# davide-coccomini/MINTIME-Multi-Identity-size-iNvariant-TIMEsformer-for-Video-Deepfake-Detection

Measured on AMD Instinct MI355X. Metric: clips/sec (8-frame, 2-identity, 224^2 crops) fwd+bwd, higher is better.
Workload: dtype f32; 1 GPU; config 3: EfficientNet-B0 + SizeInvariantTimeSformer(dim 512, depth 9, heads 8), B=32/GPU, 8 frames, 2 identities (identity-masked), 224x224 crops, random-init seeded weights (restored before every step), train-mode BN + drop-connect 0.2, step = fwd + BCE loss + bwd + SGD(lr .01, wd 1e-4); global_batch=32, frames=8, parallelism=dp1

## Files before the change

### include/mintime_hip.h

```cpp
#ifndef MINTIME_HIP_H
#define MINTIME_HIP_H
#include <stdint.h>
#ifdef __cplusplus
extern "C" {
#endif

#define MT_VERSION 122

int mt_version(void);
const char* mt_last_error(void);

int mt_set_deterministic(int on);
int mt_get_deterministic(void);
int mt_det_release(void* stream);
int mt_det_bn_sums(const float* x, const float* z, const float* mean_invstd, int64_t rows, int C, int mode, double* stats, void* stream);

typedef struct { int gin, gout, off; } mt_rowmap;

enum { MT_OP_NT = 0,
       MT_OP_NN = 1,
       MT_OP_TN = 2 };

enum { MT_PRO_NONE = 0, MT_PRO_BN_SWISH_GATE = 1, MT_PRO_BN_SWISH = 2, MT_PRO_AFFINE = 3,
       MT_PRO_BN_BWD = 4,
// ... 38 lines not shown
int mt_gemm_set_precision(int level);
int mt_gemm_get_precision(void);

int mt_split_planes(const float* src, void* planes, int64_t n, void* stream);

int64_t mt_planes_elems(int rows, int cols);

int mt_split_planes_blk(const float* src, int64_t ld, int rows, int cols, void* planes, void* stream);

int mt_split_planes_blk_multi(const void* items, int count, int64_t total_blocks, void* stream);

int mt_bn_bwd_apply_planes(const float* du, const float* z, const float* kabc, void* planes, int rows, int C, void* stream);

typedef struct {
  int op;
  int epilogue;
  int M, N, K;
  const void* a_planes;
  const void* b_planes;
  float* C; int64_t ldc;
  const float* bias;
  const float* R; int64_t ldr;
  float* C2; int64_t ldc2;
  int n_half;
  float* col_sum;
  void* c_planes;
  int split_k;
  void* sk_workspace;
  int64_t sk_workspace_bytes;
  double* stats; int stats_slots;
} mt_gemm_planes_desc;

int mt_gemm_planes(const mt_gemm_planes_desc* d, void* stream);

int mt_mul_planes(const float* x, const float* m, void* planes, float* out, int rows, int cols, void* stream);
int mt_mul_add(const float* y, const float* m, const float* r, float* out, int64_t n, void* stream);
int mt_geglu_bwd(const float* dh, const float* m, const float* u, void* du_planes, float* du, int rows, int n_half, void* stream);
int64_t mt_gemm_planes_workspace_bytes(void);
int mt_gemm_planes_set_persist(int blocks_per_cu);


int mt_layernorm_fwd(const float* x, const float* gamma, const float* beta, float* y, float* stats,
                     int rows, int dim, float eps, void* y_planes, void* stream);

int mt_embed_fwd(float* x, const float* cls, const float* pos_emb, const float* size_emb,
                 const int64_t* positions, const int32_t* sizes, int B, int F, int n, int dim, int pos_rows, int size_rows,
                 int* err_flag, void* stream);

int mt_attn_fwd(const float* qkv, float* out, float* cls_att, const uint8_t* mask, const uint8_t* ident,
                int B, int H, int F, int n, int mode, float scale, void* out_planes, void* stream);

int mt_head_fwd(const float* x, const float* gamma, const float* beta, const float* w, const float* bias,
                float* logits, int B, int N, int dim, int classes, float eps, void* stream);


int mt_stem_conv_fwd(const void* x, int x_is_u8, const float* w, float* z, double* stats, int slots, int N, int H, int W,
                     void* stream);
int mt_stem_conv_fwd_valid(const void* x, int x_is_u8, const float* w, float* z, double* stats, int slots, int N, int H, int W,
                           void* stream);

int mt_dwconv_fwd(const float* zin, const float* scale, const float* shift, const float* w, float* zout,
                  double* stats, int slots, int N, int H, int W, int C, int k, int stride, int act, void* stream);
int mt_dwconv_rc_supported(int cin, int C, int k, int stride, int H);
int mt_dwconv_fwd_rc(const float* y, const float* we, int cin, const float* scale, const float* shift, const float* w, float* zout,
                     double* stats, int slots, int N, int H, int W, int C, int k, int stride, void* stream);
int mt_dwconv_fwd_planes(const float* zin, const float* scale, const float* shift, const float* w, void* planes, int N, int H,
// ... 185 lines not shown
```

### mintime-multi-identity-size-invariant-timesformer-for-video-deepfake-detection_amd/csrc/gemm_planes.hip

```cpp
#include "../../include/mintime_hip.h"
#include "common.hpp"
#include "gemm_planes_launch.hpp"
#include "det.hpp"
#include <stdlib.h>
#include <string.h>

using namespace mt;

namespace {

__device__ __forceinline__ void to_blk_block(const float* __restrict__ src, int64_t ld, int R, int C, const PlaneRef& o, int rb, int cb, int lane) {
  const int r = rb * 32 + (lane >> 1), c = cb * 16 + (lane & 1) * 8;
  float x[8] = {0.f, 0.f, 0.f, 0.f, 0.f, 0.f, 0.f, 0.f};
  if (r < R) {
    const float* s = src + (int64_t)r * ld + c;
    if (c + 8 <= C && ((ld & 3) == 0) && (((uintptr_t)src & 15) == 0)) {
      const float4 u = *reinterpret_cast<const float4*>(s), v = *reinterpret_cast<const float4*>(s + 4);
      x[0] = u.x; x[1] = u.y; x[2] = u.z; x[3] = u.w; x[4] = v.x; x[5] = v.y; x[6] = v.z; x[7] = v.w;
    } else {
#pragma unroll
      for (int e = 0; e < 8; ++e) if (c + e < C) x[e] = s[e];
    }
  }
  planes_store8(o, r, c, x);
// ... 188 lines not shown
  bool sk = false;
  if (sk_env && d->sk_workspace && d->sk_workspace_bytes >= mt_gemm_planes_workspace_bytes() && !((uintptr_t)d->sk_workspace & 255)) {
    static const int per_cu = getenv("MT_PLANES_SK_BLOCKS") ? atoi(getenv("MT_PLANES_SK_BLOCKS")) : 2;
    int g = cu_count() * per_cu;
    g = g / 8 * 8;
    if (g > kSkMaxGrid) g = kSkMaxGrid;
    const int64_t units = (int64_t)m_tiles * n_tiles * (((d->K + 15) / 16 + 1) / 2);
    if (g >= 8 && units >= (int64_t)g * 2 && units < (1ll << 30)) {
      sk = true;
      grid = dim3((unsigned)g, 1, 1);
      a.sk_on = 1;
      a.sk_flags = reinterpret_cast<int*>(d->sk_workspace);
      a.sk_ws = reinterpret_cast<float*>(reinterpret_cast<char*>(d->sk_workspace) + kSkFlagBytes);
    }
  }
  if (!sk && !cpl && (epi == MT_EPI_STORE || epi == MT_EPI_BIAS_RES)) {
    const int per_cu = persist_blocks();
    const int g = cu_count() * per_cu / 8 * 8;
    if (per_cu > 0 && g >= 8 && m_tiles * n_tiles > g) {
      const dim3 pg((unsigned)g, 1, 1);
      const bool nt_store = op == MT_OP_NT && epi == MT_EPI_STORE, nt_bias_res = op == MT_OP_NT && epi == MT_EPI_BIAS_RES;
      const bool nn_store = op == MT_OP_NN && epi == MT_EPI_STORE;
      if (nt_store || nt_bias_res || nn_store) return launch(2, a, pg);
    }
  }
  return launch(sk ? 1 : 0, a, grid);
}

extern "C" int mt_gemm_planes(const mt_gemm_planes_desc* d, void* stream) {
  const int rc = gemm_planes_impl(d, stream);
  if (rc) { (void)mt::det_gemm_finish(nullptr, false); return rc; }
  return mt::det_gemm_finish((hipStream_t)stream, true);
}
```

### mintime-multi-identity-size-invariant-timesformer-for-video-deepfake-detection_amd/csrc/gemm_planes.hpp

```cpp
#pragma once
#include "gemm_split.hpp"
#include "planes.hpp"

#ifndef MT_PLANES_ABLATE
#define MT_PLANES_ABLATE 0
#endif
#ifndef MT_PLANES_EPI_ABLATE
#define MT_PLANES_EPI_ABLATE 0
#endif
#ifndef MT_PLANES_PRIO
#define MT_PLANES_PRIO 0
#endif

namespace mt {

typedef short s16x4_t __attribute__((ext_vector_type(4)));
enum : int { BAL_NONE = 0, BAL_PAIR = 1, BAL_PHASE = 2 };

__device__ __forceinline__ void lds_dma16_s(const void* sbase, unsigned voff, unsigned lds_byte_addr) {
  unsigned keep;
  asm volatile("s_mov_b32 %0, m0\n\ts_mov_b32 m0, %3\n\ts_nop 0\n\tglobal_load_lds_dwordx4 %1, %2\n\ts_mov_b32 m0, %0"
               : "=&s"(keep) : "v"(voff), "s"(sbase), "s"(lds_byte_addr) : "memory");
}

// ... 111 lines not shown
      }
    }
  }
}

template <int BM, int BN>
__device__ __forceinline__ void sk_tile_coords(const GemmArgs& p, int t, int& mt_, int& nt_) {
  const int n_tiles = (p.N + BN - 1) / BN, m_tiles = (p.M + BM - 1) / BM;
  if (p.group_n > 0) {
    const int q = m_tiles >> 3, r = m_tiles & 7;
    int xcd = 0, base = 0;
    for (; xcd < 7; ++xcd) {
      const int cnt = (q + (xcd < r ? 1 : 0)) * n_tiles;
      if (t < base + cnt) break;
      base += cnt;
    }
    const int rows = q + (xcd < r ? 1 : 0);
    const int row0 = xcd < r ? xcd * (q + 1) : r * (q + 1) + (xcd - r) * q;
    const int idx = t - base;
    const int per_group = rows * p.group_n;
    const int g = idx / per_group;
    const int rem = idx - g * per_group;
    const int groups = (n_tiles + p.group_n - 1) / p.group_n;
    const int gw = (g == groups - 1) ? n_tiles - g * p.group_n : p.group_n;
    const int ml = rem / gw;
    mt_ = row0 + ml;
    nt_ = g * p.group_n + (rem - ml * gw);
  } else {
    mt_ = t / n_tiles;
    nt_ = t - mt_ * n_tiles;
  }
}

template <int WAVES_M, int WAVES_N, int TM, int TN, bool AKM, bool BKM, int EPI, int STAGES, int MINW, int BAL, bool CPL = false, int SKM = 0, int NP = 3>
__global__ __launch_bounds__(WAVES_M * WAVES_N * 64, MINW)
void gemm_planes_kernel(const GemmArgs p) {
  constexpr int NW = WAVES_M * WAVES_N;
  constexpr int BM = WAVES_M * TM * 32;
  constexpr int BN = WAVES_N * TN * 32;
  constexpr int BK = 16;
  constexpr int A_PLANE = BM * 32, B_PLANE = BN * 32;
  static_assert(NP == 2 || NP == 3, "two or three pieces per operand");
  constexpr int STAGE = NP * (A_PLANE + B_PLANE);
  constexpr int PPA = A_PLANE / 1024, PPB = B_PLANE / 1024;
  constexpr int PA = NP * PPA, PB = NP * PPB;
  static_assert((PA + PB) % NW == 0, "every wavefront must issue the same number of DMA pieces");
  constexpr int IPW = (PA + PB) / NW;
  static_assert(STAGES >= 2 && STAGES <= 4, "2..4 stages");
  static_assert((!AKM || BM == 128) && (!BKM || BN == 128), "k-major images are laid out for 128-column tiles");
  constexpr bool SK = SKM == 1, PS = SKM == 2;
  static_assert(!SK || !AKM, "stream-K: forward / data-gradient forms (weight gradients split K over the grid already)");
  static_assert(!PS || (!AKM && !CPL && STAGES == 2 && EPI != EPI_GEGLU && BAL != BAL_PHASE), "persistent form: NT / NN, fp32 output, ring of two");
  constexpr bool PAIR = BAL == BAL_PAIR, PHASE = BAL == BAL_PHASE;

  extern __shared__ __attribute__((aligned(16))) unsigned char smem_pl[];
  const unsigned lds_base = (unsigned)(uintptr_t)(__attribute__((address_space(3))) unsigned char*)smem_pl;

  const int tid = threadIdx.x;
  const int lane = tid & 63;
  const int wave = __builtin_amdgcn_readfirstlane(tid >> 6);
  const int wm = wave / WAVES_N;
  const int wn = wave % WAVES_N;

  const __bf16* a_base = reinterpret_cast<const __bf16*>(p.a_planes);
  const __bf16* b_base = reinterpret_cast<const __bf16*>(p.b_planes);

  int a_frag[TM], b_frag[TN];
  {
    const int kh = lane >> 5;
// ... 350 lines not shown
        else if (has_next) issue(vn, 0, nslot);
        Frags f;
        read_frags(slot, f);
        mma(f, odd_c, 0u);
        slot = nslot;
      };
      for (int kt = 0; kt < nk; kt += 2) {
        step(kt, std::false_type{});
        if (kt + 1 >= nk) break;
        step(kt + 1, std::true_type{});
      }
      if constexpr (PAIR) {
#pragma unroll
        for (int ii = 0; ii < TM; ++ii)
#pragma unroll
          for (int jj = 0; jj < TN; ++jj)
#pragma unroll
            for (int r = 0; r < 16; ++r) acc[ii][jj][r] -= nacc[ii][jj][r];
#pragma unroll
        for (int ii = 0; ii < TM; ++ii)
#pragma unroll
          for (int jj = 0; jj < TN; ++jj) asm volatile("" : "+v"(acc[ii][jj]));
      }
      epilogue(mt_, nt_);
      if (!has_next) break;
      i = inext; mt_ = mtn; nt_ = ntn;
#pragma unroll
      for (int j = 0; j < IPW; ++j) vc[j] = vn[j];
    }
  } else if constexpr (!SK) {
    int mt_, nt_;
    int k_begin = 0, k_end = p.K;
    int split_idx = blockIdx.y;
    if (p.xcd_k) {
      const int tiles = gridDim.x, lin = blockIdx.y * gridDim.x + blockIdx.x;
      const int xcd = lin & 7, idx = lin >> 3;
      const int split = xcd + 8 * (idx / tiles), t = idx % tiles;
      const int n_tiles = (p.N + BN - 1) / BN, m_tiles = (p.M + BM - 1) / BM;
      if (m_tiles >= n_tiles) { mt_ = t / n_tiles; nt_ = t - mt_ * n_tiles; }
      else { nt_ = t / m_tiles; mt_ = t - nt_ * m_tiles; }
      k_begin = split * p.k_chunk;
      k_end = min(p.K, k_begin + p.k_chunk);
      if (k_begin >= k_end) return;
      split_idx = split;
    } else {
      if (!tile_coords<BM, BN>(p, mt_, nt_)) return;
      if (p.k_chunk > 0) {
        k_begin = blockIdx.y * p.k_chunk;
        k_end = min(p.K, k_begin + p.k_chunk);
        if (k_begin >= k_end) return;
      }
    }
    const int nk = (k_end - k_begin + BK - 1) / BK;
    if (nk <= 0) return;
    run_piece(mt_, nt_, k_begin, 0, nk);
    epilogue(mt_, nt_, split_idx);
  } else {
    const int G = gridDim.x;
    const int L = (blockIdx.x & 7) * (G >> 3) + (blockIdx.x >> 3);
    const int nkt = (p.K + BK - 1) / BK;
    const int npt = (nkt + 1) >> 1;
    const int U = ((p.N + BN - 1) / BN) * ((p.M + BM - 1) / BM) * npt;
    const int uq = U / G, ur = U % G;
    int u = L * uq + min(L, ur);
    const int u_end = u + uq + (L < ur ? 1 : 0);
    constexpr int SLAB = BM * BN;
    while (u < u_end) {
// ... 68 lines not shown
```

### mintime-multi-identity-size-invariant-timesformer-for-video-deepfake-detection_amd/lib.py

```python
import ctypes as C
import os
import subprocess
import threading

import torch

_HERE = os.path.dirname(os.path.abspath(__file__))
CSRC = os.path.join(_HERE, "csrc")
LIB_PATH = os.environ.get("MT_LIB") or os.path.join(CSRC, "libmintime_hip.so")

_lib = None

f32p = C.c_void_p
i64 = C.c_int64


class RowMap(C.Structure):
    _fields_ = [("gin", C.c_int), ("gout", C.c_int), ("off", C.c_int)]


class Conv3dDesc(C.Structure):
    _fields_ = [(n, C.c_int) for n in ("N", "T", "H", "W", "C", "To", "Ho", "Wo", "K", "kt", "kh", "kw", "st", "sh", "sw", "pt", "ph",
                                       "pw")] + [("ldx", i64), ("ldy", i64)]


class GemmDesc(C.Structure):
    _fields_ = [("op", C.c_int), ("prologue", C.c_int), ("epilogue", C.c_int),
                ("A", C.c_void_p), ("B", C.c_void_p), ("C", C.c_void_p),
                ("M", C.c_int), ("N", C.c_int), ("K", C.c_int),
                ("lda", i64), ("ldb", i64), ("ldc", i64),
                ("a_map", RowMap), ("b_map", RowMap), ("c_map", RowMap),
                ("bias", C.c_void_p), ("R", C.c_void_p), ("ldr", i64),
                ("scale", C.c_void_p), ("shift", C.c_void_p), ("gate", C.c_void_p), ("hw", C.c_int),
                ("C2", C.c_void_p), ("ldc2", i64), ("stats", C.c_void_p), ("stats_slots", C.c_int),
                ("n_half", C.c_int), ("split_k", C.c_int),
                ("A2", C.c_void_p), ("b_prologue", C.c_int), ("b_scale", C.c_void_p), ("b_shift", C.c_void_p),
                ("b_gate", C.c_void_p), ("b_hw", C.c_int),
                ("conv_H", C.c_int), ("conv_W", C.c_int), ("conv_C", C.c_int), ("conv_Ho", C.c_int), ("conv_Wo", C.c_int),
                ("conv_k", C.c_int), ("conv_stride", C.c_int), ("conv_pad", C.c_int), ("conv_act", C.c_int), ("conv_src_u8", C.c_int),
                ("col_sum", C.c_void_p), ("b_planes", C.c_void_p), ("b_plane_stride", C.c_int64),
                ("e_scale", C.c_void_p), ("e_shift", C.c_void_p), ("e_gate", C.c_void_p), ("e_dpool", C.c_void_p),
                ("e_mi", C.c_void_p), ("e_hw", C.c_int)]


class GemmPlanesDesc(C.Structure):
    _fields_ = [("op", C.c_int), ("epilogue", C.c_int), ("M", C.c_int), ("N", C.c_int), ("K", C.c_int),
                ("a_planes", C.c_void_p), ("b_planes", C.c_void_p), ("C", C.c_void_p), ("ldc", i64),
                ("bias", C.c_void_p), ("R", C.c_void_p), ("ldr", i64), ("C2", C.c_void_p), ("ldc2", i64),
                ("n_half", C.c_int), ("col_sum", C.c_void_p), ("c_planes", C.c_void_p), ("split_k", C.c_int),
                ("sk_workspace", C.c_void_p), ("sk_workspace_bytes", i64), ("stats", C.c_void_p), ("stats_slots", C.c_int)]


OP_NT, OP_NN, OP_TN = 0, 1, 2
PRO_NONE, PRO_BN_SWISH_GATE, PRO_BN_SWISH, PRO_AFFINE, PRO_BN_BWD, PRO_IM2COL = 0, 1, 2, 3, 4, 5
BPRO_NONE, BPRO_BN_SWISH_GATE, BPRO_IM2COL = 0, 1, 2
EPI_STORE, EPI_BIAS_RES, EPI_GEGLU, EPI_STATS, EPI_ATOMIC, EPI_GEGLU_BWD, EPI_ACCUM, EPI_SE_RED, EPI_ACT_BWD = 0, 1, 2, 3, 4, 5, 6, 7, 8

PROTOTYPES = {
    "mt_version": [],
    "mt_last_error": [],
    "mt_set_deterministic": [C.c_int],
    "mt_get_deterministic": [],
    "mt_det_release": [C.c_void_p],
    "mt_det_bn_sums": [f32p, f32p, f32p, i64, C.c_int, C.c_int, C.c_void_p, C.c_void_p],
    "mt_gemm": [C.POINTER(GemmDesc), C.c_void_p],
    "mt_gemm_set_split": [C.c_int],
    "mt_gemm_get_split": [],
    "mt_gemm_set_precision": [C.c_int],
    "mt_gemm_get_precision": [],
    "mt_split_planes": [f32p, C.c_void_p, C.c_int64, C.c_void_p],
    "mt_planes_elems": [C.c_int, C.c_int],
    "mt_split_planes_blk": [f32p, i64, C.c_int, C.c_int, C.c_void_p, C.c_void_p],
    "mt_split_planes_blk_multi": [C.c_void_p, C.c_int, i64, C.c_void_p],
    "mt_bn_bwd_apply_planes": [f32p, f32p, f32p, C.c_void_p, C.c_int, C.c_int, C.c_void_p],
    "mt_gemm_planes": [C.POINTER(GemmPlanesDesc), C.c_void_p],
    "mt_gemm_planes_workspace_bytes": [],
    "mt_gemm_planes_set_persist": [C.c_int],
    "mt_mul_planes": [f32p, f32p, C.c_void_p, f32p, C.c_int, C.c_int, C.c_void_p],
    "mt_mul_add": [f32p, f32p, f32p, f32p, i64, C.c_void_p],
    "mt_geglu_bwd": [f32p, f32p, f32p, C.c_void_p, f32p, C.c_int, C.c_int, C.c_void_p],
    "mt_layernorm_fwd": [f32p, f32p, f32p, f32p, f32p, C.c_int, C.c_int, C.c_float, C.c_void_p, C.c_void_p],
    "mt_embed_fwd": [f32p, f32p, f32p, f32p, C.c_void_p, C.c_void_p, C.c_int, C.c_int, C.c_int, C.c_int, C.c_int, C.c_int, C.c_void_p,
                     C.c_void_p],
    "mt_attn_fwd": [f32p, f32p, f32p, C.c_void_p, C.c_void_p, C.c_int, C.c_int, C.c_int, C.c_int, C.c_int, C.c_float,
                    C.c_void_p, C.c_void_p],
    "mt_head_fwd": [f32p, f32p, f32p, f32p, f32p, f32p, C.c_int, C.c_int, C.c_int, C.c_int, C.c_float, C.c_void_p],
    "mt_stem_conv_fwd": [C.c_void_p, C.c_int, f32p, f32p, C.c_void_p, C.c_int, C.c_int, C.c_int, C.c_int, C.c_void_p],
    "mt_stem_conv_fwd_valid": [C.c_void_p, C.c_int, f32p, f32p, C.c_void_p, C.c_int, C.c_int, C.c_int, C.c_int, C.c_void_p],
    "mt_dwconv_fwd": [f32p, f32p, f32p, f32p, f32p, C.c_void_p, C.c_int, C.c_int, C.c_int, C.c_int, C.c_int, C.c_int, C.c_int,
                      C.c_int, C.c_void_p],
    "mt_dwconv_fwd_planes": [f32p] * 4 + [C.c_void_p] + [C.c_int] * 7 + [C.c_void_p],
    "mt_dwconv_rc_supported": [C.c_int] * 5,
    "mt_dwconv_fwd_rc": [f32p, f32p, C.c_int, f32p, f32p, f32p, f32p, C.c_void_p] + [C.c_int] * 7 + [C.c_void_p],
    "mt_dwconv_bwd_rc": [f32p] * 6 + [C.c_int] + [f32p] * 4 + [C.c_void_p, C.c_int, f32p] + [C.c_int] * 7 + [C.c_void_p],
    "mt_bn_finalize": [C.c_void_p, C.c_int, C.c_double, f32p, f32p, f32p, f32p, f32p, f32p, f32p, C.c_int, C.c_float,
                       C.c_float, C.c_int, C.c_void_p],
    "mt_se_pool_parts": [C.c_int, C.c_int, C.c_int],
    "mt_se_pool_fwd": [f32p, f32p, f32p, f32p, C.c_int, C.c_int, C.c_int, C.c_int, C.c_void_p],
    "mt_se_gate_fwd": [f32p, C.c_int, f32p, f32p, f32p, f32p, f32p, f32p, f32p, C.c_int, C.c_int, C.c_int, C.c_void_p],
    "mt_bn_act_fwd": [f32p, f32p, f32p, f32p, f32p, i64, C.c_int, C.c_int, f32p, C.c_int, C.c_void_p],
    "mt_attn_aggregate": [f32p, f32p, f32p, C.c_int, C.c_int, C.c_int, C.c_float, C.c_void_p],
    "mt_build_clip_inputs": [C.c_void_p] * 8 + [C.c_int] * 5 + [C.c_void_p],
    "mt_layernorm_bwd": [f32p, f32p, f32p, f32p, f32p, f32p, f32p, C.c_int, C.c_int, C.c_int, f32p, C.c_int, f32p, C.c_void_p],
    "mt_layernorm_bwd_rows": [f32p, f32p, f32p, f32p, f32p, f32p, C.c_int, C.c_int, C.c_void_p, C.c_void_p],
    "mt_layernorm_bwd_cols": [f32p, f32p, f32p, f32p, f32p, f32p, f32p, C.c_int, C.c_int, C.c_int, C.c_void_p],
    "mt_layernorm_bwd_rows_blocks": [C.c_int],
    "mt_layernorm_bwd_rows_sums": [f32p, f32p, f32p, f32p, f32p, f32p, C.c_int, C.c_int, C.c_void_p, f32p, C.c_int, C.c_void_p],
    "mt_layernorm_bwd_cols_reduce": [f32p, C.c_int, C.c_int, f32p, f32p, f32p, C.c_void_p],
# ... 227 lines not shown

def gemm_planes(op, a_planes, b_planes, M, N, K, Cout=None, ldc=0, epilogue=EPI_STORE, bias=None, R=None, ldr=0, C2=None, ldc2=0,
                n_half=0, col_sum=None, c_planes=None, split_k=0, streamk=None, stats=None, stats_slots=0):
    d = GemmPlanesDesc()
    if streamk is None:
        streamk = os.environ.get("MT_PLANES_STREAMK", "0") != "0"
    if streamk and op != OP_TN:
        ws = streamk_workspace(a_planes.device)
        if ws is not None:
            d.sk_workspace, d.sk_workspace_bytes = ptr(ws), ws.numel()
    d.op, d.epilogue, d.M, d.N, d.K = op, epilogue, M, N, K
    d.a_planes, d.b_planes, d.C, d.ldc = ptr(a_planes), ptr(b_planes), ptr(Cout), ldc
    d.bias, d.R, d.ldr, d.C2, d.ldc2 = ptr(bias), ptr(R), ldr, ptr(C2), ldc2
    d.n_half, d.col_sum, d.c_planes, d.split_k = n_half, ptr(col_sum), ptr(c_planes), split_k
    d.stats, d.stats_slots = ptr(stats), stats_slots
    if recording() is not None:
        if op == OP_TN:
            tag_next(TAG_WGRAD, 2.0 * M * N * K)
        elif epilogue == EPI_GEGLU:
            tag_next(TAG_FF1, 2.0 * M * N * K)
    prof = PROFILE
    if prof is not None:
        for pr in prof:
            if "match_planes" in pr and pr["match_planes"](d):
                e0, e1 = torch.cuda.Event(enable_timing=True), torch.cuda.Event(enable_timing=True)
                e0.record()
                check(get().mt_gemm_planes(C.byref(d), stream_ptr()), "mt_gemm_planes")
                e1.record()
                pr["events"].append((e0, e1, 2.0 * M * N * K))
                return
    check(get().mt_gemm_planes(C.byref(d), stream_ptr()), "mt_gemm_planes")


def gemm_split_enabled() -> bool:
    return bool(get().mt_gemm_get_split())


def check(rc, what):
    if rc != 0:
        msg = get().mt_last_error()
        raise MintimeHipError(f"{what} failed ({rc}): {msg.decode() if msg else ''}")


def stream_ptr():
    return C.c_void_p(torch.cuda.current_stream().cuda_stream)


def ptr(t):
    if t is None:
        return None
    if not t.is_cuda:
        raise MintimeHipError("libmintime_hip takes device pointers only; got a CPU tensor (no CPU fallback exists)")
    rec = getattr(_REC, "plan", None)
    if rec is not None:
        rec.keep[id(t)] = t
    return C.c_void_p(t.data_ptr())


_REC = threading.local()

TAG_WGRAD, TAG_FF1, TAG_DWCONV_DGRAD = 1, 2, 3


def recording():
    return getattr(_REC, "plan", None)

# ... 255 lines not shown
```

### mintime-multi-identity-size-invariant-timesformer-for-video-deepfake-detection_amd/tsf_engine.py

```python
import ctypes as C
import os
import types

import torch

from . import arch
from . import lib as L
from . import plans, tsf_planes
from .tsf_backward import tsf_backward


def _as_tokens(x):
    b, f, c, h, w = x.shape
    t = x.permute(0, 1, 3, 4, 2)
    if not t.is_contiguous():
        t = t.contiguous()
    return t.reshape(b * f * h * w, c)


class _Aux:

    def __init__(self, model, x, mask, identities_mask, size_embedding, positions):
        dev = x.device
        b, f = x.shape[0], x.shape[1]
# ... 172 lines not shown
            L.gemm(L.OP_NT, hbuf, w2, x_new, M, D, 4 * D, 4 * D, 4 * D, D, epilogue=L.EPI_ATOMIC, bias=b2, split_k=5)
        else:
            x_new = _new(dev, B, N, D) if save else x
            L.gemm(L.OP_NT, hbuf, w2, x_new, M, D, 4 * D, 4 * D, 4 * D, D, epilogue=L.EPI_BIAS_RES, bias=b2, R=x, ldr=D)
        if save:
            rec[2] = dict(x=x, xn=xn, stats=stats, u=u, h=hbuf)
            saved["layers"].append(rec)
        x = x_new
    g, b_, w_h, b_h = next(it), next(it), next(it), next(it)
    logits = _new(dev, B, model.num_classes)
    L.check(lib.mt_head_fwd(L.ptr(x), L.ptr(g), L.ptr(b_), L.ptr(w_h), L.ptr(b_h), L.ptr(logits), B, x.shape[1], D, model.num_classes,
                            eps, st), "mt_head_fwd")
    if save:
        saved["x_final"] = x
    return logits, s_att, t_att, saved


_AUX = ("mask", "ident", "sizes", "positions")


class _TSFFunction(torch.autograd.Function):
    @staticmethod
    def forward(ctx, model, aux, dims, feat, *params):
        B, F, n, grad_on = dims
        dims = (B, F, n)
        save = grad_on and any(ctx.needs_input_grad)
        ctx.model, ctx.dims, ctx.params = model, dims, params
        planes = tsf_planes.eligible(model, B * (1 + F * n), save)
        stream = key = None
        if planes and save and not tsf_planes.dropout_active(model):
            stream = torch.cuda.current_stream(feat.device).cuda_stream
            key = ("tsf", B, F, n, feat.dtype, model.training, model.require_attention, L.deterministic(),
                   tuple(ctx.needs_input_grad[3:]), stream, os.environ.get("MT_PLANES_STREAMK", "0"),
                   tuple(getattr(aux, nm) is None for nm in _AUX))

        def body(ins, plan):
            a = aux if plan is None else types.SimpleNamespace(err=aux.err, **{nm: ins["aux_" + nm] for nm in _AUX})
            if planes:
                logits, s_att, t_att, saved = tsf_planes.tsf_forward_planes(model, ins["feat"], a, params, B, F, n, save)
            elif tsf_planes.dropout_active(model):
                raise NotImplementedError("attn-dropout / ff-dropout > 0 in train mode runs on the plane path only (MT_TSF_PLANES=1, "
                                          "MT_GEMM_SPLIT=1, no MT_TSF_PRUNE_LAST / MT_WGRAD_DEFER, not under stream capture)")
            else:
                logits, s_att, t_att, saved = tsf_forward(model, ins["feat"], a, params, B, F, n, save)
            if saved is not None:
                saved.update(feat=ins["feat"], aux=a)
            return (logits, s_att, t_att), saved
        inputs = {"feat": feat, **{"aux_" + nm: getattr(aux, nm) for nm in _AUX}}
        logits, s_att, t_att = plans.forward(ctx, model, key, stream, params, inputs, body, clone_outputs=True,
                                             after_run=lambda np_: _publish_index_flag(aux.err))
        if model.require_attention:
            ctx.mark_non_differentiable(s_att, t_att)
            return logits, s_att, t_att
        return (logits,)

    @staticmethod
    def backward(ctx, dlogits, *unused):
        s = ctx.saved
        need_df, need_dp = ctx.needs_input_grad[3], ctx.needs_input_grad[4:]

        def body(g, keep_saved, plan):
            if s.get("planes"):
                dfeat, dparams = tsf_planes.tsf_backward_planes(ctx.model, s["feat"], s["aux"], ctx.params, ctx.dims, s, g, need_df,
                                                                need_dp, keep_saved=keep_saved, plan=plan)
            else:
                dfeat, dparams = tsf_backward(ctx.model, s["feat"], s["aux"], ctx.params, ctx.dims, s, g, need_df, need_dp)
            return (dfeat,), dparams
# ... 64 lines not shown
```

### mintime-multi-identity-size-invariant-timesformer-for-video-deepfake-detection_amd/tsf_planes.py

```python
import os

import torch

from . import arch
from . import lib as L
from . import plans

LN_FOLD = os.environ.get("MT_LN_FOLD", "1") != "0"

_SEL = (2, 3, 7, 8, 12, 14)


def eligible(model, M, save):
    if os.environ.get("MT_TSF_PLANES", "1") == "0" or not L.gemm_split_enabled():
        return False
    if os.environ.get("MT_TSF_PRUNE_LAST", "0") != "0" or os.environ.get("MT_WGRAD_DEFER", "0") != "0":
        return False
    if torch.cuda.is_current_stream_capturing() and save:
        return False
    D, inner = model.dim, model.heads * model.dim_head
    return (M >= 512 or dropout_active(model)) and D % 16 == 0 and inner % 16 == 0 and model.dim_head == 64


def dropout_active(model):
# ... 105 lines not shown
        g, b_, w1, b1, w2, b2 = next(it), next(it), next(it), next(it), next(it), next(it)
        if save:
            xn_p, h_p, stats = L.planes_empty(M, D, dev), L.planes_empty(M, 4 * D, dev), _new(dev, M, 2)
            u = _new(dev, M, 8 * D)
        else:
            stats, u = None, None
        L.check(lib.mt_layernorm_fwd(L.ptr(x), L.ptr(g), L.ptr(b_), None, L.ptr(stats), M, D, eps, L.ptr(xn_p), st), "mt_layernorm_fwd")
        dm = None
        if p_ff > 0.0:
            dm = _dropout_mult(model, (M, 4 * D), p_ff, dev)
            h = _new(dev, M, 4 * D)
            L.gemm_planes(L.OP_NT, xn_p, wp[(li, 12)], M, 8 * D, D, epilogue=L.EPI_GEGLU, bias=b1, C2=u, ldc2=8 * D, n_half=4 * D,
                          Cout=h, ldc=4 * D)
            L.check(lib.mt_mul_planes(L.ptr(h), L.ptr(dm), L.ptr(h_p), None, M, 4 * D, st), "mt_mul_planes")
            del h
        else:
            L.gemm_planes(L.OP_NT, xn_p, wp[(li, 12)], M, 8 * D, D, epilogue=L.EPI_GEGLU, bias=b1, C2=u, ldc2=8 * D, n_half=4 * D,
                          c_planes=h_p)
        x_new = _new(dev, B, N, D) if save else x
        L.gemm_planes(L.OP_NT, h_p, wp[(li, 14)], M, D, 4 * D, Cout=x_new, ldc=D, epilogue=L.EPI_BIAS_RES, bias=b2, R=x, ldr=D)
        if save:
            rec[2] = dict(x=x, stats=stats, xn_p=xn_p, u=u, h_p=h_p, dm=dm)
            saved["layers"].append(rec)
        x = x_new
    g, b_, w_h, b_h = next(it), next(it), next(it), next(it)
    logits = _new(dev, B, model.num_classes)
    L.check(lib.mt_head_fwd(L.ptr(x), L.ptr(g), L.ptr(b_), L.ptr(w_h), L.ptr(b_h), L.ptr(logits), B, x.shape[1], D, model.num_classes,
                            eps, st), "mt_head_fwd")
    if save:
        saved["x_final"] = x
    return logits, s_att, t_att, saved


def tsf_backward_planes(model, feat, aux, params, dims, saved, dlogits, need_dfeat, need_dparams, keep_saved=False, plan=None):
    lib = L.get()
    st = L.stream_ptr()
    dev = feat.device
    B, F, n = dims
    D, H, dh, C_in = model.dim, model.heads, model.dim_head, model.channels
    inner = H * dh
    N = 1 + F * n
    M = B * N
    eps = arch.LN_EPS
    scale = float(dh) ** -0.5
    wp = saved["wp"]
    grads, flat_grads = L.zero_grads(list(params), with_flat=True)
    P = list(params)
    idx = len(P)

    def take(k):
        nonlocal idx
        idx -= k
        return idx

    side = L.SideStream(dev, hold=True)

    def wgrad(a_p, b_p, out, M_, N_, bias_src=None, bias_out=None):
        def run():
            L.gemm_planes(L.OP_TN, a_p, b_p, M_, N_, M, Cout=out, ldc=N_, epilogue=L.EPI_ATOMIC)
            if bias_out is not None:
                L.check(lib.mt_colsum(L.ptr(bias_src), D, L.RowMap(0, 0, 0), M, D, L.ptr(bias_out), L.stream_ptr()), "mt_colsum")
        return side.launch(run, reads=(a_p, b_p, bias_src))

    def ln_bwd(dxn_, r_, g_, dx_cur, i_g, tgt, skip):
        dx_new = torch.empty_like(dx_cur)
        dx_p = L.planes_empty(M, D, dev)
        x_, st_ = r_["x"], r_["stats"]
        if LN_FOLD and D <= 512:
            nb = lib.mt_layernorm_bwd_rows_blocks(M)
            part = _new(dev, nb, 3, D)
            L.check(lib.mt_layernorm_bwd_rows_sums(L.ptr(dxn_), L.ptr(x_), L.ptr(st_), L.ptr(g_), L.ptr(dx_new), L.ptr(dx_cur), M, D,
                                                   L.ptr(dx_p), L.ptr(part), skip, st), "mt_layernorm_bwd_rows_sums")
            side.launch(lambda: L.check(lib.mt_layernorm_bwd_cols_reduce(L.ptr(part), nb, D, L.ptr(grads[i_g]), L.ptr(grads[i_g + 1]),
                                                                         L.ptr(tgt), L.stream_ptr()), "mt_layernorm_bwd_cols_reduce"),
                        reads=(part,))
            return dx_new, dx_p
        L.check(lib.mt_layernorm_bwd_rows(L.ptr(dxn_), L.ptr(x_), L.ptr(st_), L.ptr(g_), L.ptr(dx_new), L.ptr(dx_cur), M, D,
                                          L.ptr(dx_p), st), "mt_layernorm_bwd_rows")
        side.launch(lambda: L.check(lib.mt_layernorm_bwd_cols(L.ptr(dxn_), L.ptr(x_), L.ptr(st_), L.ptr(dx_new), L.ptr(grads[i_g]),
                                                              L.ptr(grads[i_g + 1]), L.ptr(tgt), skip, M, D, L.stream_ptr()),
                                    "mt_layernorm_bwd_cols"), reads=(dxn_, x_, st_, dx_new))
        return dx_new, dx_p

    i0 = take(4)
    g, b_, w_h, b_h = P[i0:i0 + 4]
    dx = L.zeros((B, N, D), torch.float32, dev)
    L.check(lib.mt_head_bwd(L.ptr(dlogits), L.ptr(saved["x_final"]), L.ptr(g), L.ptr(b_), L.ptr(w_h), L.ptr(dx), L.ptr(grads[i0]),
                            L.ptr(grads[i0 + 1]), L.ptr(grads[i0 + 2]), L.ptr(grads[i0 + 3]), B, N, D, model.num_classes, eps,
                            st), "mt_head_bwd")
    dx2 = dx.view(M, D)
    dx_p = L.split_planes_blk(dx2, M, D)
    do = torch.empty(M, inner, dtype=torch.float32, device=dev)
    dqkv = torch.empty(M, 3 * inner, dtype=torch.float32, device=dev)

    for li in reversed(range(model.depth)):
        rec = saved["layers"][li]
        i0 = take(6)
        g, b_, w1, b1, w2, b2 = P[i0:i0 + 6]
        r = rec[2]
        du_p = L.planes_empty(M, 8 * D, dev)
        dxn = torch.empty(M, D, dtype=torch.float32, device=dev)
        last = li == model.depth - 1
        wgrad(dx_p, r["h_p"], grads[i0 + 4], D, 4 * D, bias_src=dx2 if last else None, bias_out=grads[i0 + 5] if last else None)
        if r.get("dm") is not None:
            dh, du_f = torch.empty(M, 4 * D, dtype=torch.float32, device=dev), torch.empty(M, 8 * D, dtype=torch.float32, device=dev)
            L.gemm_planes(L.OP_NN, dx_p, wp[(li, 14)], M, 4 * D, D, Cout=dh, ldc=4 * D)
            L.check(lib.mt_geglu_bwd(L.ptr(dh), L.ptr(r["dm"]), L.ptr(r["u"]), L.ptr(du_p), L.ptr(du_f), M, 4 * D, st), "mt_geglu_bwd")
            side.launch(lambda du_f=du_f, out=grads[i0 + 3]: L.check(lib.mt_colsum(L.ptr(du_f), 8 * D, L.RowMap(0, 0, 0), M, 8 * D,
                                                                                 L.ptr(out), L.stream_ptr()), "mt_colsum"), reads=(du_f,))
            del dh
        else:
            L.gemm_planes(L.OP_NN, dx_p, wp[(li, 14)], M, 4 * D, D, epilogue=L.EPI_GEGLU_BWD, C2=r["u"], ldc2=8 * D, n_half=4 * D,
                          col_sum=grads[i0 + 3], c_planes=du_p)
        wgrad(du_p, r["xn_p"], grads[i0 + 2], 8 * D, D)
        L.gemm_planes(L.OP_NN, du_p, wp[(li, 12)], M, D, 8 * D, Cout=dxn, ldc=D)
        dx2, dx_p = ln_bwd(dxn, r, g, dx2, i0, None if rec[1].get("dm") is not None else grads[i0 - 1], 0)
        if not keep_saved:
            r.clear()
        for mode in (1, 0):
            i0 = take(5)
            g, b_, w_qkv, w_o, b_o = P[i0:i0 + 5]
            r = rec[mode]
            dxn = torch.empty(M, D, dtype=torch.float32, device=dev)
            dy_p = dx_p
            if r.get("dm") is not None:
                dy_p = L.planes_empty(M, D, dev)
                dy_f = torch.empty(M, D, dtype=torch.float32, device=dev)
                L.check(lib.mt_mul_planes(L.ptr(dx2), L.ptr(r["dm"]), L.ptr(dy_p), L.ptr(dy_f), M, D, st), "mt_mul_planes")
                side.launch(lambda dy_f=dy_f, out=grads[i0 + 4]: L.check(lib.mt_colsum(L.ptr(dy_f), D, L.RowMap(0, 0, 0), M, D, L.ptr(out),
                                                                                     L.stream_ptr()), "mt_colsum"), reads=(dy_f,))
            wgrad(dy_p, r["o_p"], grads[i0 + 3], D, inner)
            L.gemm_planes(L.OP_NN, dy_p, wp[(li, 8 if mode == 1 else 3)], M, inner, D, Cout=do, ldc=inner)
            dqkv_p = L.planes_empty(M, 3 * inner, dev)
            L.check(lib.mt_attn_bwd(L.ptr(r["qkv"]), L.ptr(do), L.ptr(dqkv), L.ptr(aux.mask), L.ptr(aux.ident), B, H, F, n, mode,
                                    scale, L.ptr(dqkv_p), st), "mt_attn_bwd")
            wgrad(dqkv_p, r["xn_p"], grads[i0 + 2], 3 * inner, D)
            L.gemm_planes(L.OP_NN, dqkv_p, wp[(li, 7 if mode == 1 else 2)], M, D, 3 * inner, Cout=dxn, ldc=D)
            if mode == 0 and li == 0:
                tgt, skip = grads[1], N
            elif mode == 1 and rec[0].get("dm") is not None:
                tgt, skip = None, 0
            else:
                tgt, skip = grads[i0 - 1], 0
            dx2, dx_p = ln_bwd(dxn, r, g, dx2, i0, tgt, skip)
            if not keep_saved:
                r.clear()
        side.release_point()

    i0 = take(5)
    w_pe, b_pe, cls, pos_w, size_w = P[i0:i0 + 5]
    dx = dx2.view(B, N, D)
    L.check(lib.mt_embed_bwd(L.ptr(dx), L.ptr(grads[i0 + 2]), L.ptr(grads[i0 + 3]), L.ptr(grads[i0 + 4]), L.ptr(aux.positions),
                             L.ptr(aux.sizes), B, F, n, D, pos_w.shape[0], size_w.shape[0] if size_w is not None else 0, st),
            "mt_embed_bwd")
    tok_map = (F * n, N, 1)
    Mt = B * F * n
    side.launch(lambda: L.gemm(L.OP_TN, dx2, feat, grads[i0], D, C_in, Mt, D, C_in, C_in, epilogue=L.EPI_ATOMIC, split_k=0, a_map=tok_map),
                reads=(dx2, feat))
    dfeat = None
    if need_dfeat:
        dfeat = torch.empty(Mt, C_in, dtype=torch.float32, device=dev)
        L.gemm(L.OP_NN, dx2, w_pe, dfeat, Mt, C_in, D, D, C_in, C_in, a_map=tok_map)
    side.wait()
    assert idx == 0
    if plan is not None:
        plan.extra["flat_grads"] = flat_grads
    L.grads_ready(model, params, flat_grads)
    return dfeat, [gr if gneed else None for gneed, gr in zip(need_dparams, grads)]
```

Baseline: 720.4 clips/s.

## Group transformer weight-gradient GEMMs into single split-K grouped launches

```diff
diff --git a/include/mintime_hip.h b/include/mintime_hip.h
--- a/include/mintime_hip.h
+++ b/include/mintime_hip.h
@@ -94,6 +94,21 @@
 } mt_gemm_planes_desc;
 
 int mt_gemm_planes(const mt_gemm_planes_desc* d, void* stream);
+
+#define MT_GEMM_PLANES_GROUP_MAX 8
+typedef struct {
+  int count;
+  int splits;
+  struct {
+    int M, N, K;
+    const void* a_planes;
+    const void* b_planes;
+    float* C; int64_t ldc;
+  } p[MT_GEMM_PLANES_GROUP_MAX];
+} mt_gemm_planes_group_desc;
+int mt_gemm_planes_tn_group(const mt_gemm_planes_group_desc* d, void* stream);
+int mt_gemm_planes_tn_group_blocks(const mt_gemm_planes_group_desc* d);
+int mt_gemm_planes_tn_group_decode(const mt_gemm_planes_group_desc* d, int block, int* out);
 
 int mt_mul_planes(const float* x, const float* m, void* planes, float* out, int rows, int cols, void* stream);
 int mt_mul_add(const float* y, const float* m, const float* r, float* out, int64_t n, void* stream);
diff --git a/mintime-multi-identity-size-invariant-timesformer-for-video-deepfake-detection_amd/csrc/gemm_planes.hip b/mintime-multi-identity-size-invariant-timesformer-for-video-deepfake-detection_amd/csrc/gemm_planes.hip
--- a/mintime-multi-identity-size-invariant-timesformer-for-video-deepfake-detection_amd/csrc/gemm_planes.hip
+++ b/mintime-multi-identity-size-invariant-timesformer-for-video-deepfake-detection_amd/csrc/gemm_planes.hip
@@ -244,3 +244,96 @@
   if (rc) { (void)mt::det_gemm_finish(nullptr, false); return rc; }
   return mt::det_gemm_finish((hipStream_t)stream, true);
 }
+
+
+static int group_prepare(const mt_gemm_planes_group_desc* d, PlaneGroupArgs& g) {
+  if (!d) return fail(MT_ERR_ARG, "mt_gemm_planes_tn_group: null descriptor");
+  if (d->count < 1 || d->count > MT_GEMM_PLANES_GROUP_MAX)
+    return fail(MT_ERR_ARG, "mt_gemm_planes_tn_group: %d problems (1 .. %d per launch)", d->count, MT_GEMM_PLANES_GROUP_MAX);
+  static_assert(MT_GEMM_PLANES_GROUP_MAX == kPlaneGroupMax, "the C ABI's group size is the kernel's");
+  memset(&g, 0, sizeof(g));
+  g.count = d->count;
+  g.K = d->p[0].K;
+  int tiles = 0;
+  for (int i = 0; i < d->count; ++i) {
+    const auto& q = d->p[i];
+    if (q.M <= 0 || q.N <= 0 || q.K <= 0) return fail(MT_ERR_ARG, "mt_gemm_planes_tn_group: problem %d has a bad shape %d %d %d", i, q.M, q.N, q.K);
+    if (q.K != g.K) return fail(MT_ERR_ARG, "mt_gemm_planes_tn_group: problem %d has K = %d, problem 0 has %d (one K per group)", i, q.K, g.K);
+    if (q.ldc < q.N) return fail(MT_ERR_ARG, "mt_gemm_planes_tn_group: problem %d: ldc %lld < N %d", i, (long long)q.ldc, q.N);
+    PlaneGroupProblem& o = g.pr[i];
+    o.M = q.M; o.N = q.N; o.ldc = q.ldc;
+    o.a_pstride = mt_planes_elems(q.K, q.M); o.lda = (q.M + 15) >> 4;
+    o.b_pstride = mt_planes_elems(q.K, q.N); o.ldb = (q.N + 15) >> 4;
+    if (6 * o.a_pstride > 0xFFFFFFFFll || 6 * o.b_pstride > 0xFFFFFFFFll)
+      return fail(MT_ERR_UNSUPPORTED, "mt_gemm_planes_tn_group: problem %d: an operand's planes span %lld bytes (> 4 GB: 32-bit DMA offsets)", i,
+                  (long long)(6 * (o.a_pstride > o.b_pstride ? o.a_pstride : o.b_pstride)));
+    g.first[i] = tiles;
+    tiles += ((q.M + 127) / 128) * ((q.N + 127) / 128);
+    if (tiles > (1 << 20)) return fail(MT_ERR_UNSUPPORTED, "mt_gemm_planes_tn_group: more than 2^20 output tiles");
+  }
+  for (int i = d->count; i <= kPlaneGroupMax; ++i) g.first[i] = tiles;
+  g.tiles = tiles;
+  int splits = d->splits;
+  if (splits <= 0) {
+    splits = (1280 + tiles - 1) / tiles;
+    const int max_splits = g.K / 256 > 0 ? g.K / 256 : 1;
+    if (splits > max_splits) splits = max_splits;
+  }
+  splits = splits <= 2 ? splits : splits <= 4 ? 4 : (splits + 7) / 8 * 8;
+  if (splits > 64) splits = 64;
+  g.splits = splits;
+  int chunk = (g.K + splits - 1) / splits;
+  g.k_chunk = (chunk + 15) / 16 * 16;
+  g.per_xcd = splits >= 8 ? 0 : (tiles + 8 / splits - 1) / (8 / splits);
+  return 0;
+}
+
+extern "C" int mt_gemm_planes_tn_group_blocks(const mt_gemm_planes_group_desc* d) {
+  PlaneGroupArgs g;
+  if (int rc = group_prepare(d, g)) return rc;
+  return planes_group_blocks(g);
+}
+
+extern "C" int mt_gemm_planes_tn_group_decode(const mt_gemm_planes_group_desc* d, int block, int* out) {
+  PlaneGroupArgs g;
+  if (int rc = group_prepare(d, g)) return rc;
+  if (!out || block < 0 || block >= planes_group_blocks(g)) return fail(MT_ERR_ARG, "mt_gemm_planes_tn_group_decode: block %d outside the grid", block);
+  int prob = 0, mt_ = 0, nt_ = 0, split = 0;
+  if (!planes_group_decode(g, block, prob, mt_, nt_, split)) return 0;
+  const int k_begin = split * g.k_chunk, k_end = g.K < k_begin + g.k_chunk ? g.K : k_begin + g.k_chunk;
+  if (k_begin >= k_end) return 0;
+  out[0] = prob; out[1] = mt_; out[2] = nt_; out[3] = split; out[4] = k_begin; out[5] = k_end;
+  return 1;
+}
+
+extern "C" int mt_gemm_planes_tn_group(const mt_gemm_planes_group_desc* d, void* stream) {
+  PlaneGroupArgs g;
+  if (int rc = group_prepare(d, g)) return rc;
+  for (int i = 0; i < d->count; ++i) {
+    const auto& q = d->p[i];
+    if (!q.a_planes || !q.b_planes || !q.C) return fail(MT_ERR_ARG, "mt_gemm_planes_tn_group: problem %d has a null pointer", i);
+    if (((uintptr_t)q.a_planes & 15) || ((uintptr_t)q.b_planes & 15))
+      return fail(MT_ERR_ARG, "mt_gemm_planes_tn_group: problem %d: planes must be 16-byte aligned", i);
+    if ((uintptr_t)q.C & 3) return fail(MT_ERR_ARG, "mt_gemm_planes_tn_group: problem %d: C must be 4-byte aligned", i);
+    g.pr[i].a_planes = q.a_planes; g.pr[i].b_planes = q.b_planes; g.pr[i].C = q.C;
+  }
+  if (det_enabled() || matmul_precision() == MT_PRECISION_HIGH) {
+    for (int i = 0; i < d->count; ++i) {
+      const auto& q = d->p[i];
+      mt_gemm_planes_desc s;
+      memset(&s, 0, sizeof(s));
+      s.op = MT_OP_TN; s.epilogue = MT_EPI_ATOMIC; s.M = q.M; s.N = q.N; s.K = q.K;
+      s.a_planes = q.a_planes; s.b_planes = q.b_planes; s.C = q.C; s.ldc = q.ldc;
+      if (int rc = mt_gemm_planes(&s, stream)) return rc;
+    }
+    return 0;
+  }
+  auto k = gemm_planes_kernel<2, 2, 2, 2, true, true, EPI_ATOMIC, 2, 3, BAL_NONE, false, 0, 3, PlaneGroupArgs>;
+  constexpr size_t lds = (size_t)2 * 3 * (128 + 128) * 32;
+  {
+    hipError_t e = ensure_dynamic_lds(reinterpret_cast<const void*>(k), lds);
+    if (e != hipSuccess) return fail(MT_ERR_LAUNCH, "mt_gemm_planes_tn_group: cannot reserve %zu B of LDS: %s", lds, hipGetErrorString(e));
+  }
+  hipLaunchKernelGGL(k, dim3((unsigned)planes_group_blocks(g)), dim3(256), lds, (hipStream_t)stream, g);
+  return check_launch("mt_gemm_planes_tn_group");
+}
diff --git a/mintime-multi-identity-size-invariant-timesformer-for-video-deepfake-detection_amd/csrc/gemm_planes.hpp b/mintime-multi-identity-size-invariant-timesformer-for-video-deepfake-detection_amd/csrc/gemm_planes.hpp
--- a/mintime-multi-identity-size-invariant-timesformer-for-video-deepfake-detection_amd/csrc/gemm_planes.hpp
+++ b/mintime-multi-identity-size-invariant-timesformer-for-video-deepfake-detection_amd/csrc/gemm_planes.hpp
@@ -167,9 +167,83 @@
   }
 }
 
-template <int WAVES_M, int WAVES_N, int TM, int TN, bool AKM, bool BKM, int EPI, int STAGES, int MINW, int BAL, bool CPL = false, int SKM = 0, int NP = 3>
+struct PlaneBlockWork { int mt, nt, k_begin, k_end, split; };
+
+constexpr int kPlaneGroupMax = 8;
+struct PlaneGroupProblem {
+  const void* a_planes; const void* b_planes; float* C;
+  int64_t ldc, a_pstride, b_pstride;
+  int M, N, lda, ldb;
+};
+struct PlaneGroupArgs {
+  PlaneGroupProblem pr[kPlaneGroupMax];
+  int first[kPlaneGroupMax + 1];
+  int count, K, k_chunk;
+  int splits;
+  int tiles;
+  int per_xcd;
+};
+__host__ __device__ inline int planes_group_blocks(const PlaneGroupArgs& g) { return g.splits >= 8 ? g.tiles * g.splits : 8 * g.per_xcd; }
+
+__host__ __device__ inline bool planes_group_decode(const PlaneGroupArgs& g, int lin, int& prob, int& mt_, int& nt_, int& split) {
+  const int xcd = lin & 7, idx = lin >> 3;
+  int t;
+  if (g.splits >= 8) {
+    split = xcd + 8 * (idx / g.tiles);
+    t = idx % g.tiles;
+    if (split >= g.splits) return false;
+  } else {
+    split = xcd & (g.splits - 1);
+    if (idx >= g.per_xcd) return false;
+    t = (xcd / g.splits) * g.per_xcd + idx;
+    if (t >= g.tiles) return false;
+  }
+  prob = 0;
+#pragma unroll
+  for (int i = 1; i < kPlaneGroupMax; ++i)
+    if (i < g.count && g.first[i] <= t) prob = i;
+  t -= g.first[prob];
+  const int m_tiles = (g.pr[prob].M + 127) / 128, n_tiles = (g.pr[prob].N + 127) / 128;
+  if (m_tiles >= n_tiles) { mt_ = t / n_tiles; nt_ = t - mt_ * n_tiles; }
+  else { nt_ = t / m_tiles; mt_ = t - nt_ * m_tiles; }
+  return true;
+}
+
+template <bool GRP> struct PlaneGroupBlock {
+  PlaneBlockWork w;
+  __device__ __forceinline__ const GemmArgs& args(const GemmArgs& ka) const { return ka; }
+};
+template <> struct PlaneGroupBlock<true> {
+  PlaneBlockWork w;
+  GemmArgs p;
+  __device__ __forceinline__ bool decode(const PlaneGroupArgs& g, int lin) {
+    int prob;
+    if (!planes_group_decode(g, lin, prob, w.mt, w.nt, w.split)) return false;
+    w.k_begin = w.split * g.k_chunk;
+    w.k_end = min(g.K, w.k_begin + g.k_chunk);
+    if (w.k_begin >= w.k_end) return false;
+    const PlaneGroupProblem& q = g.pr[prob];
+    p = GemmArgs{};
+    p.C = q.C; p.M = q.M; p.N = q.N; p.K = g.K; p.ldc = q.ldc;
+    p.a_planes = q.a_planes; p.a_pstride = q.a_pstride; p.lda = q.lda;
+    p.b_planes = q.b_planes; p.b_pstride = q.b_pstride; p.ldb = q.ldb;
+    p.hw = 1; p.b_hw = 1; p.e_hw = 1; p.stats_slots = 1;
+    p.k_chunk = g.k_chunk;
+    return true;
+  }
+  __device__ __forceinline__ const GemmArgs& args(const PlaneGroupArgs&) const { return p; }
+};
+
+template <int WAVES_M, int WAVES_N, int TM, int TN, bool AKM, bool BKM, int EPI, int STAGES, int MINW, int BAL, bool CPL = false, int SKM = 0, int NP = 3,
+          class KA = GemmArgs>
 __global__ __launch_bounds__(WAVES_M * WAVES_N * 64, MINW)
-void gemm_planes_kernel(const GemmArgs p) {
+void gemm_planes_kernel(const KA ka) {
+  constexpr bool GRP = std::is_same<KA, PlaneGroupArgs>::value;
+  static_assert(!GRP || (AKM && BKM && EPI == EPI_ATOMIC && SKM == 0 && !CPL), "grouped launches: the weight-gradient form");
+  PlaneGroupBlock<GRP> grp;
+  if constexpr (GRP) { if (!grp.decode(ka, (int)blockIdx.x)) return; }
+  const GemmArgs& p = grp.args(ka);
+  const PlaneBlockWork& w = grp.w;
   constexpr int NW = WAVES_M * WAVES_N;
   constexpr int BM = WAVES_M * TM * 32;
   constexpr int BN = WAVES_N * TN * 32;
@@ -586,7 +660,9 @@
     int mt_, nt_;
     int k_begin = 0, k_end = p.K;
     int split_idx = blockIdx.y;
-    if (p.xcd_k) {
+    if constexpr (GRP) {
+      mt_ = w.mt; nt_ = w.nt; k_begin = w.k_begin; k_end = w.k_end; split_idx = w.split;
+    } else if (p.xcd_k) {
       const int tiles = gridDim.x, lin = blockIdx.y * gridDim.x + blockIdx.x;
       const int xcd = lin & 7, idx = lin >> 3;
       const int split = xcd + 8 * (idx / tiles), t = idx % tiles;
diff --git a/mintime-multi-identity-size-invariant-timesformer-for-video-deepfake-detection_amd/lib.py b/mintime-multi-identity-size-invariant-timesformer-for-video-deepfake-detection_amd/lib.py
--- a/mintime-multi-identity-size-invariant-timesformer-for-video-deepfake-detection_amd/lib.py
+++ b/mintime-multi-identity-size-invariant-timesformer-for-video-deepfake-detection_amd/lib.py
@@ -49,6 +49,18 @@
                 ("bias", C.c_void_p), ("R", C.c_void_p), ("ldr", i64), ("C2", C.c_void_p), ("ldc2", i64),
                 ("n_half", C.c_int), ("col_sum", C.c_void_p), ("c_planes", C.c_void_p), ("split_k", C.c_int),
                 ("sk_workspace", C.c_void_p), ("sk_workspace_bytes", i64), ("stats", C.c_void_p), ("stats_slots", C.c_int)]
+
+
+GROUP_MAX = 8
+
+
+class GemmPlanesGroupProblem(C.Structure):
+    _fields_ = [("M", C.c_int), ("N", C.c_int), ("K", C.c_int), ("a_planes", C.c_void_p), ("b_planes", C.c_void_p),
+                ("C", C.c_void_p), ("ldc", i64)]
+
+
+class GemmPlanesGroupDesc(C.Structure):
+    _fields_ = [("count", C.c_int), ("splits", C.c_int), ("p", GemmPlanesGroupProblem * GROUP_MAX)]
 
 
 OP_NT, OP_NN, OP_TN = 0, 1, 2
@@ -74,6 +86,9 @@
     "mt_split_planes_blk_multi": [C.c_void_p, C.c_int, i64, C.c_void_p],
     "mt_bn_bwd_apply_planes": [f32p, f32p, f32p, C.c_void_p, C.c_int, C.c_int, C.c_void_p],
     "mt_gemm_planes": [C.POINTER(GemmPlanesDesc), C.c_void_p],
+    "mt_gemm_planes_tn_group": [C.POINTER(GemmPlanesGroupDesc), C.c_void_p],
+    "mt_gemm_planes_tn_group_blocks": [C.POINTER(GemmPlanesGroupDesc)],
+    "mt_gemm_planes_tn_group_decode": [C.POINTER(GemmPlanesGroupDesc), C.c_int, C.POINTER(C.c_int)],
     "mt_gemm_planes_workspace_bytes": [],
     "mt_gemm_planes_set_persist": [C.c_int],
     "mt_mul_planes": [f32p, f32p, C.c_void_p, f32p, C.c_int, C.c_int, C.c_void_p],
@@ -367,6 +382,43 @@
     check(get().mt_gemm_planes(C.byref(d), stream_ptr()), "mt_gemm_planes")
 
 
+def group_desc(shapes, splits):
+    if len(shapes) > GROUP_MAX:
+        raise MintimeHipError(f"a grouped launch takes at most {GROUP_MAX} problems, got {len(shapes)}")
+    d = GemmPlanesGroupDesc()
+    d.count, d.splits = len(shapes), splits
+    for q, (M, N, K) in zip(d.p, shapes):
+        q.M, q.N, q.K, q.ldc = M, N, K, N
+    return d
+
+
+def gemm_planes_tn_group(problems, K, splits):
+    if len(problems) > GROUP_MAX:
+        raise MintimeHipError(f"a grouped launch takes at most {GROUP_MAX} problems, got {len(problems)}")
+    d = GemmPlanesGroupDesc()
+    d.count, d.splits = len(problems), splits
+    work = 0.0
+    for q, (a_p, b_p, M, N, Cout, ldc) in zip(d.p, problems):
+        q.M, q.N, q.K = M, N, K
+        q.a_planes, q.b_planes, q.C, q.ldc = ptr(a_p), ptr(b_p), ptr(Cout), ldc
+        work += 2.0 * M * N * K
+    if recording() is not None:
+        tag_next(TAG_WGRAD, work)
+    prof = PROFILE
+    if prof is not None:
+        as_tn = GemmPlanesDesc()
+        as_tn.op, as_tn.epilogue, as_tn.K = OP_TN, EPI_ATOMIC, K
+        for pr in prof:
+            if "match_planes" in pr and pr["match_planes"](as_tn):
+                e0, e1 = torch.cuda.Event(enable_timing=True), torch.cuda.Event(enable_timing=True)
+                e0.record()
+                check(get().mt_gemm_planes_tn_group(C.byref(d), stream_ptr()), "mt_gemm_planes_tn_group")
+                e1.record()
+                pr["events"].append((e0, e1, work))
+                return
+    check(get().mt_gemm_planes_tn_group(C.byref(d), stream_ptr()), "mt_gemm_planes_tn_group")
+
+
 def gemm_split_enabled() -> bool:
     return bool(get().mt_gemm_get_split())
 
diff --git a/mintime-multi-identity-size-invariant-timesformer-for-video-deepfake-detection_amd/tsf_engine.py b/mintime-multi-identity-size-invariant-timesformer-for-video-deepfake-detection_amd/tsf_engine.py
--- a/mintime-multi-identity-size-invariant-timesformer-for-video-deepfake-detection_amd/tsf_engine.py
+++ b/mintime-multi-identity-size-invariant-timesformer-for-video-deepfake-detection_amd/tsf_engine.py
@@ -228,7 +228,7 @@
             stream = torch.cuda.current_stream(feat.device).cuda_stream
             key = ("tsf", B, F, n, feat.dtype, model.training, model.require_attention, L.deterministic(),
                    tuple(ctx.needs_input_grad[3:]), stream, os.environ.get("MT_PLANES_STREAMK", "0"),
-                   tuple(getattr(aux, nm) is None for nm in _AUX))
+                   tuple(getattr(aux, nm) is None for nm in _AUX), tsf_planes.wgrad_group_key())
 
         def body(ins, plan):
             a = aux if plan is None else types.SimpleNamespace(err=aux.err, **{nm: ins["aux_" + nm] for nm in _AUX})
diff --git a/mintime-multi-identity-size-invariant-timesformer-for-video-deepfake-detection_amd/tsf_planes.py b/mintime-multi-identity-size-invariant-timesformer-for-video-deepfake-detection_amd/tsf_planes.py
--- a/mintime-multi-identity-size-invariant-timesformer-for-video-deepfake-detection_amd/tsf_planes.py
+++ b/mintime-multi-identity-size-invariant-timesformer-for-video-deepfake-detection_amd/tsf_planes.py
@@ -161,6 +161,14 @@
     return logits, s_att, t_att, saved
 
 
+WGRAD_GROUPED = True
+WGRAD_GROUP_SPLITS = {"ff": 4, "attn": 4, "pair": 8}
+
+
+def wgrad_group_key():
+    return WGRAD_GROUPED, tuple(sorted(WGRAD_GROUP_SPLITS.items()))
+
+
 def tsf_backward_planes(model, feat, aux, params, dims, saved, dlogits, need_dfeat, need_dparams, keep_saved=False, plan=None):
     lib = L.get()
     st = L.stream_ptr()
@@ -190,6 +198,30 @@
             if bias_out is not None:
                 L.check(lib.mt_colsum(L.ptr(bias_src), D, L.RowMap(0, 0, 0), M, D, L.ptr(bias_out), L.stream_ptr()), "mt_colsum")
         return side.launch(run, reads=(a_p, b_p, bias_src))
+
+    dropout = any(sub.get("dm") is not None for rec_ in saved["layers"] for sub in rec_.values())
+    grouped = WGRAD_GROUPED and not dropout and not L.deterministic() and L.get_matmul_precision() == "highest"
+    pend = []
+
+    def wgrad_later(a_p, b_p, out, M_, N_):
+        if grouped:
+            pend.append((a_p, b_p, M_, N_, out, N_))
+        else:
+            wgrad(a_p, b_p, out, M_, N_)
+
+    def wgrad_flush(kind):
+        if not pend:
+            return
+        group = list(pend)
+        pend.clear()
+
+        def run():
+            try:
+                L.gemm_planes_tn_group(group, M, WGRAD_GROUP_SPLITS[kind])
+            except L.MintimeHipError:
+                for a_p, b_p, M_, N_, out, ldc in group:
+                    L.gemm_planes(L.OP_TN, a_p, b_p, M_, N_, M, Cout=out, ldc=ldc, epilogue=L.EPI_ATOMIC)
+        side.launch(run, reads=tuple(t for q in group for t in q[:2]))
 
     def ln_bwd(dxn_, r_, g_, dx_cur, i_g, tgt, skip):
         dx_new = torch.empty_like(dx_cur)
@@ -230,7 +262,10 @@
         du_p = L.planes_empty(M, 8 * D, dev)
         dxn = torch.empty(M, D, dtype=torch.float32, device=dev)
         last = li == model.depth - 1
-        wgrad(dx_p, r["h_p"], grads[i0 + 4], D, 4 * D, bias_src=dx2 if last else None, bias_out=grads[i0 + 5] if last else None)
+        if last:
+            wgrad(dx_p, r["h_p"], grads[i0 + 4], D, 4 * D, bias_src=dx2, bias_out=grads[i0 + 5])
+        else:
+            wgrad_later(dx_p, r["h_p"], grads[i0 + 4], D, 4 * D)
         if r.get("dm") is not None:
             dh, du_f = torch.empty(M, 4 * D, dtype=torch.float32, device=dev), torch.empty(M, 8 * D, dtype=torch.float32, device=dev)
             L.gemm_planes(L.OP_NN, dx_p, wp[(li, 14)], M, 4 * D, D, Cout=dh, ldc=4 * D)
@@ -241,7 +276,8 @@
         else:
             L.gemm_planes(L.OP_NN, dx_p, wp[(li, 14)], M, 4 * D, D, epilogue=L.EPI_GEGLU_BWD, C2=r["u"], ldc2=8 * D, n_half=4 * D,
                           col_sum=grads[i0 + 3], c_planes=du_p)
-        wgrad(du_p, r["xn_p"], grads[i0 + 2], 8 * D, D)
+        wgrad_later(du_p, r["xn_p"], grads[i0 + 2], 8 * D, D)
+        wgrad_flush("ff")
         L.gemm_planes(L.OP_NN, du_p, wp[(li, 12)], M, D, 8 * D, Cout=dxn, ldc=D)
         dx2, dx_p = ln_bwd(dxn, r, g, dx2, i0, None if rec[1].get("dm") is not None else grads[i0 - 1], 0)
         if not keep_saved:
@@ -258,12 +294,17 @@
                 L.check(lib.mt_mul_planes(L.ptr(dx2), L.ptr(r["dm"]), L.ptr(dy_p), L.ptr(dy_f), M, D, st), "mt_mul_planes")
                 side.launch(lambda dy_f=dy_f, out=grads[i0 + 4]: L.check(lib.mt_colsum(L.ptr(dy_f), D, L.RowMap(0, 0, 0), M, D, L.ptr(out),
                                                                                      L.stream_ptr()), "mt_colsum"), reads=(dy_f,))
-            wgrad(dy_p, r["o_p"], grads[i0 + 3], D, inner)
+            wg = wgrad if (li == 0 and mode == 0) else wgrad_later
+            wg(dy_p, r["o_p"], grads[i0 + 3], D, inner)
             L.gemm_planes(L.OP_NN, dy_p, wp[(li, 8 if mode == 1 else 3)], M, inner, D, Cout=do, ldc=inner)
             dqkv_p = L.planes_empty(M, 3 * inner, dev)
             L.check(lib.mt_attn_bwd(L.ptr(r["qkv"]), L.ptr(do), L.ptr(dqkv), L.ptr(aux.mask), L.ptr(aux.ident), B, H, F, n, mode,
                                     scale, L.ptr(dqkv_p), st), "mt_attn_bwd")
-            wgrad(dqkv_p, r["xn_p"], grads[i0 + 2], 3 * inner, D)
+            wg(dqkv_p, r["xn_p"], grads[i0 + 2], 3 * inner, D)
+            if mode == 0:
+                wgrad_flush("attn")
+            elif li == 0:
+                wgrad_flush("pair")
             L.gemm_planes(L.OP_NN, dqkv_p, wp[(li, 7 if mode == 1 else 2)], M, D, 3 * inner, Cout=dxn, ldc=D)
             if mode == 0 and li == 0:
                 tgt, skip = grads[1], N
```

Result: no change. 722.6 clips/s (median of 6 runs) (+0.3%).
